# LSimon95/megatts2

Measured on AMD Instinct MI355X. Metric: mel-frames/sec (whole node), higher is better.
Workload: dtype f32; 1 GPU; C3: B=32/GPU x 1 GPU, Np=70, Tp=431, Tm=431; stages vqpe+mrte+adm+plm+decoder+vocoder; forced durations; weights=synthetic (name-seeded), parallelism=dp1 (utterance shards, one RCCL all-gather of mels per step)

## Files before the change

### megatts2_amd/csrc/capi.inc

```

namespace mt2 {
extern thread_local std::string g_last_error;
void finalize_model(mt2_model& m);
}

using namespace mt2;

#define MT2_API_BEGIN try {
#define MT2_API_END                                 \
    ::CallScope::verdict_of_open_call();            \
    return 0;                                       \
    }                                               \
    catch (const std::exception& e) {               \
        g_last_error = e.what();                    \
        return -1;                                  \
    }                                               \
    catch (...) {                                   \
        g_last_error = "unknown error";             \
        return -1;                                  \
    }

enum Need { NEED_G = 1, NEED_ADM = 2, NEED_PLM = 4, NEED_VOC = 8 };
static void require_ready(mt2_model* m, int need = 0) {
    MT2_REQUIRE(m != nullptr, "null model handle");
// ... 235 lines not shown
            f += R + 14 * R * ch;
        }
        f += R + 4ll * B + 64;
    }
    *bytes = (size_t)f * sizeof(float) + (size_t)400 * 256 + ((size_t)8 << 20);
    MT2_API_END
}

static int* option_slot(mt2_model* m, const std::string& n) {
    if (n == "ar_groups") return &m->ar_groups;
    if (n == "adm_groups") return &m->adm_groups;
    if (n == "plm_groups") return &m->plm_groups;
    if (n == "force_gemm_config") return &m->opts.force_cfg;
    if (n == "t_ks4") return &m->opts.t_ks4;
    if (n == "t_ks2") return &m->opts.t_ks2;
    if (n == "t32") return &m->opts.t32;
    if (n == "t32x32") return &m->opts.t32x32;
    if (n == "t_x6_256") return &m->opts.t_x6_256;
    if (n == "t_x6_128") return &m->opts.t_x6_128;
    if (n == "t_x3h_128") return &m->opts.t_x3h_128;
    if (n == "x3h") return &m->opts.x3h;
    if (n == "x6_ks") return &m->opts.x6_ks;
    if (n == "voc_streams") return &m->opts.voc_streams;
    if (n == "ldr_prio") return &m->opts.ldr_prio;
    if (n == "skinny_rows") return &m->opts.skinny_rows;
    if (n == "skinny_nw") return &m->opts.skinny_nw;
    if (n == "skinny_pairs") return &m->opts.skinny_pairs;
    if (n == "attn_lds_min") return &m->opts.attn_lds_min;
    if (n == "attn_x6_min") return &m->opts.attn_x6_min;
    if (n == "ln_pairs_adm") return &m->opts.ln_pairs_adm;
    if (n == "ln_pairs_maxm") return &m->opts.ln_pairs_maxm;
    if (n == "a_planes") return &m->opts.a_planes;
    return nullptr;
}
static bool* option_flag(mt2_model* m, const std::string& n) {
    if (n == "splitk") return &m->opts.splitk;
    if (n == "stage_markers") return &m->opts.markers;
    if (n == "win_conv") return &m->opts.win_conv;
    if (n == "x6_conv") return &m->opts.x6_conv;
    if (n == "x6_gemm") return &m->opts.x6_gemm;
    if (n == "skinny_tm") return &m->opts.skinny_tm;
    if (n == "ldr64") return &m->opts.ldr64;
    return nullptr;
}
int mt2_set_option(mt2_model* m, const char* name, int value) {
    MT2_API_BEGIN
// ... 935 lines not shown
```

### megatts2_amd/csrc/gemm_f32.hip

```cpp
#include "gemm_common.h"

#include <algorithm>
#include <atomic>
#include <cstdio>
#include <utility>
#include <vector>

namespace mt2 {

constexpr int LS = 36;

template <int BM, int BN, int WGM, int WGN>
__global__ __launch_bounds__(WGM* WGN * 64) void gemm_f32_kernel(GemmP p) {
    constexpr int NT = WGM * WGN * 64;
    constexpr int WTM = BM / WGM, WTN = BN / WGN;
    constexpr int TM = WTM / 32, TN = WTN / 32;
    constexpr int A_IT = BM * 8 / NT, B_IT = BN * 8 / NT;
    constexpr int ROWS_PER_IT = NT / 8;
    static_assert(BM * 8 % NT == 0 && BN * 8 % NT == 0, "tile/thread mismatch");
    static_assert(WTM % 32 == 0 && WTN % 32 == 0, "wave tile must be 32x32 MFMA tiles");

    extern __shared__ __attribute__((aligned(16))) float smem[];
    const int tid = threadIdx.x, lane = tid & 63, wave = tid >> 6;
    const int wm = wave / WGN, wn = wave % WGN;
// ... 1410 lines not shown
    { 32, 32, 512, 0, "skinny32_f32", { nullptr, nullptr, nullptr, nullptr, nullptr } },
    { 64, 32, 512, 0, "skinny64_f32", { nullptr, nullptr, nullptr, nullptr, nullptr } },
    { 32, 32, 512, 0, "skinnytm32_f32", { nullptr, nullptr, nullptr, nullptr, nullptr } },
    { 64, 32, 512, 0, "skinnytm64_f32", { nullptr, nullptr, nullptr, nullptr, nullptr } },
    MT2_RETIRED("x3hldr128x128_4x2+4_s3"),
    MT2_RETIRED("x3hldr128x128_4x2+4_s4"),
    MT2_RETIRED("x3hldr128x128_2x2+4_s3"),
    MT2_RETIRED("x3hldr128x128_2x2+4_s4"),
    MT2_X3HK(X3H_KS_32x64_K4, 32, 64, 1, 2, 4, 8, 2),
    MT2_X3HK(X3H_KS_64x64_K2, 64, 64, 2, 2, 2, 8, 3),
    MT2_X3HK(X3H_KS_32x32_K8, 32, 32, 1, 1, 8, 8, 2),
    MT2_X3HW(X3H_WIN_256x32, 1, 256, 32, 8, 1, 4, 4),
    MT2_X3HW(X3H_WIN_256x64, 2, 256, 64, 8, 1, 4, 4),
    MT2_X3HW(X3H_WIN_128x128, 4, 128, 128, 4, 2, 3, 4),
    MT2_RETIRED("x3hldr128x128_4x2+4_s4c2"),
    MT2_RETIRED("x3hldr128x128_2x2+4_s4c2"),
    MT2_X3HL(X3H_LDR_128x128, 128, 128, 4, 2, 4, 4, true),
    MT2_RETIRED("x3hldr128x128_4x2+4_s3xc"),
    MT2_RETIRED("x3hldr128x128_2x2+4_s4xc"),
};
constexpr int kSkinny32 = 87, kSkinny64 = 88, kSkinnyTm32 = 89, kSkinnyTm64 = 90;
constexpr int kNumCfgs = sizeof(kCfgs) / sizeof(kCfgs[0]);

int gemm_trace_shapes(EngineOpts& o, char* buf, int cap, int top) {
    struct Agg { int cfg, M, N, K, g; long long n; double ms, fl; };
    std::vector<Agg> v;
    for (auto& r : o.trace) {
        float dt = 0.f;
        if (hipEventSynchronize(r.e1) != hipSuccess || hipEventElapsedTime(&dt, r.e0, r.e1) != hipSuccess) return -1;
        bool found = false;
        for (auto& a : v)
            if (a.cfg == r.cfg && a.M == r.M && a.N == r.N && a.K == r.K && a.g == r.groups) {
                ++a.n; a.ms += dt; a.fl += r.flops; found = true;
                break;
            }
        if (!found) v.push_back({r.cfg, r.M, r.N, r.K, r.groups, 1, (double)dt, r.flops});
    }
    std::sort(v.begin(), v.end(), [](const Agg& a, const Agg& b) { return a.ms > b.ms; });
    int off = 0;
    for (int i = 0; i < (int)v.size() && i < top; ++i) {
        const Agg& a = v[i];
        const int w = snprintf(buf + off, cap - off, "%s %d %d %d %d %lld %.3f %.2f\n", kCfgs[a.cfg].name, a.M, a.N, a.K, a.g,
                               a.n, a.ms, a.fl / (a.ms > 0 ? a.ms : 1e-9) / 1e9);
        if (w < 0 || w >= cap - off) break;
        off += w;
    }
    return off;
}

int gemm_num_configs() { return kNumCfgs; }
const char* gemm_config_name(int idx) { return idx >= 0 && idx < kNumCfgs ? kCfgs[idx].name : ""; }

static std::atomic<unsigned long long> g_attr_done[kNumCfgs][6];

int gemm_trace_collect(EngineOpts& o, int cap, const char** names, int64_t* launches, double* flops, double* ms) {
    o.trace_on = false;
    auto& tr = o.trace;
    int n = 0;
    std::vector<std::pair<double, double>> iv;
    double fl_all = 0.0;
    bool ok = true;
    for (int i = 0; i < kNumCfgs && n < cap && ok; ++i) {
        int64_t cnt = 0;
        double fl = 0.0, t = 0.0;
        for (auto& r : tr) {
            if (r.cfg != i) continue;
            float dt = 0.f, t0 = 0.f;
            if (hipEventSynchronize(r.e1) != hipSuccess || hipEventElapsedTime(&dt, r.e0, r.e1) != hipSuccess ||
                hipEventElapsedTime(&t0, tr.front().e0, r.e0) != hipSuccess) { ok = false; break; }
            iv.emplace_back((double)t0, (double)t0 + dt);
            ++cnt; fl += r.flops; t += dt;
        }
        if (cnt == 0) continue;
        names[n] = kCfgs[i].name; launches[n] = cnt; flops[n] = fl; ms[n] = t;
        fl_all += fl;
        ++n;
    }
    if (ok && n < cap && !iv.empty()) {
        std::sort(iv.begin(), iv.end());
        double uni = 0.0, lo = iv[0].first, hi = iv[0].second;
        for (auto& x : iv) {
            if (x.first > hi) { uni += hi - lo; lo = x.first; hi = x.second; }
            else if (x.second > hi) hi = x.second;
        }
        uni += hi - lo;
        names[n] = "union"; launches[n] = (int64_t)iv.size(); flops[n] = fl_all; ms[n] = uni;
        ++n;
    }
    for (auto& r : tr) { (void)hipEventDestroy(r.e0); (void)hipEventDestroy(r.e1); }
    tr.clear();
    return ok ? n : -1;
}


static bool win_eligible(const GemmP& p) {
    return p.taps >= 2 && !p.rowbase && p.a_mul == 1 && p.groups == 1 && p.N == p.Cin &&
           (p.Cin == 32 || p.Cin == 64 || p.Cin == 128) && (p.taps - 1) * p.dil <= 64 && p.pro_act < PRO_LN;
// ... 185 lines not shown
    if (opts) { opts->last_stat_nt = p.stat_nt; opts->last_stat_w = p.stat_w; }
    const int tiles = ((p.M + c->bm - 1) / c->bm) * ((p.N + c->bn - 1) / c->bn);
    p.epi_t4 = o.epi_t4 ? 1 : 0;
    p.ldr_prio = o.ldr_prio;
    p.ldr64 = o.ldr64 ? 1 : 0;
    dim3 grid(tiles, 1, p.groups), block(c->threads);
    if (opts) opts->last_cfg = c->name;
    if (opts && opts->trace_on) {
        TraceRec r;
        r.cfg = idx;
        r.flops = 2.0 * p.M * p.N * p.K * p.groups;
        r.M = p.M; r.N = p.N; r.K = p.K; r.groups = p.groups;
        if (hipEventCreate(&r.e0) != hipSuccess || hipEventCreate(&r.e1) != hipSuccess) return hipErrorUnknown;
        (void)hipEventRecord(r.e0, s);
        hipLaunchKernelGGL(fn, grid, block, lds, s, p);
        (void)hipEventRecord(r.e1, s);
        opts->trace.push_back(r);
        return hipGetLastError();
    }
    hipLaunchKernelGGL(fn, grid, block, lds, s, p);
    return hipGetLastError();
}


}
```

### megatts2_amd/csrc/gemm_x3h.hip

```cpp
#include "gemm_common.h"

#include <atomic>

#ifndef MT2_X3H_ABLATE
#define MT2_X3H_ABLATE 0
#endif
#define MT2_ABL_NOINGEST (MT2_X3H_ABLATE == 2 || MT2_X3H_ABLATE == 5 || MT2_X3H_ABLATE == 6 || MT2_X3H_ABLATE == 7)
#define MT2_ABL_NOSPLIT (MT2_X3H_ABLATE == 3 || MT2_X3H_ABLATE == 5 || MT2_X3H_ABLATE == 6)
#define MT2_ABL_NOBARRIER (MT2_X3H_ABLATE == 6 || MT2_X3H_ABLATE == 7)
#ifdef MT2_X3H_NO_BUFFER_LOADS
#define MT2_BUFFER_LOADS false
#else
#define MT2_BUFFER_LOADS true
#endif

namespace mt2 {

typedef _Float16 f16x8 __attribute__((ext_vector_type(8)));
typedef _Float16 f16x2 __attribute__((ext_vector_type(2)));
typedef float f32x2 __attribute__((ext_vector_type(2)));
typedef unsigned u32x4 __attribute__((ext_vector_type(4)));

constexpr float kX3hLoScale = 2048.0f, kX3hLoInv = 1.0f / 2048.0f, kX3hMaxIn = 65504.0f;

// ... 735 lines not shown
    } else {
        float out[16];
#pragma unroll
        for (int e = 0; e < 16; ++e) out[e] = acc[e] * inv_s;
        if (lnx) {
            const int n = n0 + wn * 32 + (lane & 31);
            const float s_n = n < p.N ? p.ln_g[n] : 0.0f;
#pragma unroll
            for (int e = 0; e < 16; ++e) {
                const int rr = (e & 3) + 8 * (e >> 2) + 4 * half;
                out[e] = __shfl(ln_rs, rr) * (out[e] - __shfl(ln_mu, rr) * s_n);
            }
        }
        if (PRO == PRO_LNX && p.stat_out) epilogue_pre<16, PRO == PRO_LNX>(p, out, pre, g, m0 + wm * 32, n0 + wn * 32, lane, 0);
        else epilogue_pre<16>(p, out, pre, g, m0 + wm * 32, n0 + wn * 32, lane, 0);
    }
    if (probe) {
        __builtin_amdgcn_s_waitcnt(0);
        const unsigned long long t_end = __builtin_amdgcn_s_memrealtime();
        if (lane == 0) p.dbg[10] = t_end - t_loop_end;
    }
}

template <int QS, int BM, int BN, int WGM, int WGN, int NST, int PRO, int NL>
__global__ __launch_bounds__((WGM * WGN + NL) * 64) void conv_win_x3h_kernel(GemmP p) {
    constexpr int NW = WGM * WGN;
    constexpr int WTM = BM / WGM, WTN = BN / WGN;
    constexpr int TM = WTM / 32, TN = WTN / 32;
    constexpr int BPIECES = BN / 8;
    constexpr int NI = NL;
    constexpr int B_IT = (BPIECES + NI - 1) / NI;
    constexpr int STAGE_B = B_IT * NI * 1024;
    static_assert(NL > 0 && WTM % 32 == 0 && WTN % 32 == 0 && NST >= 3 && (NST - 2) * B_IT < 64 && BN == 32 * QS, "config");

    extern __shared__ __attribute__((aligned(16))) float smem[];
    const int tid = threadIdx.x, lane = tid & 63;
    const int wave_all = __builtin_amdgcn_readfirstlane(tid >> 6);
    const bool loader = wave_all >= NW;
    const int wave = loader ? wave_all - NW : wave_all;
    const int wm = wave / WGN, wn = wave % WGN;
    const int taps = p.taps, dil = p.dil;
    const int WR = BM + (taps - 1) * dil, WRp = (WR + 7) & ~7;
    char* ring = reinterpret_cast<char*>(smem);
    float* win = smem + NST * STAGE_B / 4;

    const int ntm = (p.M + BM - 1) / BM;
    const int bid = blockIdx.x;
    const int xcd = bid & 7, qq = ntm >> 3, rr = ntm & 7;
    const int tile = (xcd < rr ? xcd * (qq + 1) : rr * (qq + 1) + (xcd - rr) * qq) + (bid >> 3);
    const int m0 = tile * BM;

    const float* __restrict__ X = p.X;
    const char* __restrict__ Wh = reinterpret_cast<const char*>(p.Wh);
    const long long zoff_x = (const float*)g_zero16 - X;
    const long long zoff_w = (const char*)g_zero16 - Wh;
    const int ldx = p.ldx, Rx = p.Rx, Kt = p.K;

    {
        const int lrow = lane >> 3;
        const int ppq = WRp >> 3, pieces = QS * ppq;
        const int row_first = m0 + p.shift0;
        for (int pc = wave_all; pc < pieces; pc += NW + NL) {
            const int q = pc / ppq, r8 = pc - q * ppq;
            const int row = r8 * 8 + lrow;
            const int grow = row_first + row;
            const int slot = (lane & 7) ^ ((row >> 1) & 7);
            const bool ok = (row < WR) & ((unsigned)grow < (unsigned)Rx);
            const long long off = ok ? (long long)grow * ldx + q * 32 + slot * 4 : zoff_x;
            __builtin_amdgcn_global_load_lds((const __attribute__((address_space(1))) void*)(X + off),
                                             (__attribute__((address_space(3))) void*)(win + (q * WRp + r8 * 8) * 32), 16, 0, 0);
        }
    }
    const int nk = Kt / 32;
    long long wofs[B_IT];
#pragma unroll
    for (int j = 0; j < B_IT; ++j) {
        const int pc = j * NI + wave;
        const int n = pc * 8 + (lane >> 3);
        const int sl = (lane & 7) ^ ((n >> 1) & 7);
        wofs[j] = (pc < BPIECES && n < p.N) ? (long long)n * p.wh_ldb + sl * 16 : -1;
    }
    constexpr unsigned kOut = 0x80000000u;
    const bool fast32 = MT2_BUFFER_LOADS && !p.ldr64 && (long long)p.N * p.wh_ldb < 0x7fffffffll;
    const __amdgpu_buffer_rsrc_t rs_w = __builtin_amdgcn_make_buffer_rsrc(const_cast<char*>(Wh), 0, (int)kOut, 0x00020000);
    unsigned vob[B_IT];
#pragma unroll
    for (int j = 0; j < B_IT; ++j) vob[j] = wofs[j] >= 0 ? (unsigned)wofs[j] : kOut;
    auto issue = [&](int c, int st) __attribute__((always_inline)) {
        char* Bs = ring + st * STAGE_B + wave * 1024;
        if (fast32) {
#pragma unroll
            for (int j = 0; j < B_IT; ++j)
                __builtin_amdgcn_raw_ptr_buffer_load_lds(rs_w, (__attribute__((address_space(3))) void*)(Bs + j * NI * 1024), 16, (int)vob[j], c * 128, 0, 0);
            return;
        }
#pragma unroll
        for (int j = 0; j < B_IT; ++j) {
            const long long off = wofs[j] >= 0 ? wofs[j] + (long long)c * 128 : zoff_w;
            __builtin_amdgcn_global_load_lds((const __attribute__((address_space(1))) void*)(Wh + off),
                                             (__attribute__((address_space(3))) void*)(Bs + j * NI * 1024), 16, 0, 0);
        }
    };
    if (loader) {
        loader_priority(p.ldr_prio);
#pragma unroll
        for (int st = 0; st < NST - 1; ++st)
            if (st < nk) issue(st, st);
        if (nk >= NST - 1) wait_vmcnt<(NST - 1) * B_IT>();
        else wait_vmcnt<0>();
    } else {
        wait_vmcnt<0>();
    }
    float amax = 0.0f;
    {
        constexpr int NT = (NW + NL) * 64;
        constexpr int MAXT = (QS * (BM + 64) * 4 + NT - 1) / NT;
        const unsigned lds_w = (unsigned)(unsigned long long)(__attribute__((address_space(3))) float*)win;
        const int ntask = QS * WRp * 4;
        f32x4 in[MAXT][2];
        __builtin_amdgcn_s_barrier();
        asm volatile("" ::: "memory");
#pragma unroll
        for (int u = 0; u < MAXT; ++u) {
            const int t = tid + u * NT;
            const int tt = t < ntask ? t : 0;
            const int rbk = tt >> 2, j = tt & 3;
            const int row = rbk % WRp;
            const int swz = (row >> 1) & 7;
            const unsigned base = lds_w + (unsigned)rbk * 128;
            in[u][0] = lds_read_b128(base + (unsigned)(((2 * j) ^ swz) * 16));
            in[u][1] = lds_read_b128(base + (unsigned)(((2 * j + 1) ^ swz) * 16));
        }
        asm volatile("s_waitcnt lgkmcnt(0)" ::: "memory");
#pragma unroll
// ... 4 lines not shown
#pragma unroll
        for (int u = 0; u < MAXT; ++u) {
            const int t = tid + u * NT;
            if (t < ntask) {
                const int rbk = t >> 2, j = t & 3;
                const int row = rbk % WRp;
                const int swz = (row >> 1) & 7;
                u32x4 ph, pl;
                split2_f16<PRO>(in[u][0], in[u][1], slope0, ph, pl, amax);
                char* dst = reinterpret_cast<char*>(win) + (size_t)rbk * 128;
                *reinterpret_cast<u32x4*>(dst + ((j ^ swz) * 16)) = ph;
                *reinterpret_cast<u32x4*>(dst + (((4 + j) ^ swz) * 16)) = pl;
            }
        }
        asm volatile("s_waitcnt lgkmcnt(0)" ::: "memory");
    }
    if (p.x3h_flag != nullptr && __builtin_amdgcn_ballot_w64(amax >= kX3hMaxIn) != 0ull && lane == 0) atomicOr(p.x3h_flag, 1);
    if (loader) {
        static_assert(NST >= 3, "cross-chunk form: chunk c-1 is still being read at barrier c");
        for (int c = 0; c < nk; ++c) {
            if (c == 0) { if (NST - 2 < nk) wait_vmcnt<(NST - 2) * B_IT>(); else wait_vmcnt<0>(); }
            else if (c + NST - 3 < nk) wait_vmcnt<(NST - 3) * B_IT>();
            else wait_vmcnt<0>();
            __builtin_amdgcn_s_barrier();
            if (c >= 1 && c + NST - 2 < nk) issue(c + NST - 2, (c + NST - 2) % NST);
        }
        return;
    }
    float inv_s[TN];
#pragma unroll
    for (int j = 0; j < TN; ++j) {
        const int n = wn * WTN + j * 32 + (lane & 31);
        inv_s[j] = p.wh_inv[n < p.N ? n : 0];
    }

    f32x16 acc[TM][TN], acl[TM][TN];
#pragma unroll
    for (int i = 0; i < TM; ++i)
#pragma unroll
        for (int j = 0; j < TN; ++j)
#pragma unroll
            for (int e = 0; e < 16; ++e) { acc[i][j][e] = 0.0f; acl[i][j][e] = 0.0f; }

    const int half = lane >> 5;
    const unsigned lds_ring = (unsigned)(unsigned long long)(__attribute__((address_space(3))) char*)ring;
    const unsigned lds_win = (unsigned)(unsigned long long)(__attribute__((address_space(3))) float*)win;
    const int nrow = wn * WTN + (lane & 31);
    const unsigned b_lane = lds_ring + nrow * 128;
    const int swzb = (nrow >> 1) & 7;
    unsigned koffb[2][2];
#pragma unroll
    for (int b = 0; b < 2; ++b) {
        koffb[b][0] = (unsigned)(((b * 2 + half) ^ swzb) * 16);
        koffb[b][1] = (unsigned)(((4 + b * 2 + half) ^ swzb) * 16);
    }
    const int arow0 = wm * WTM + (lane & 31);

    constexpr int N1 = 2 * TM + 2 * TN;
    static_assert(N1 <= 15, "lgkmcnt is four bits wide");
    u32x4 ra[2][TM][2];
    u32x4 rb[2][2][TN];
    auto fetch_a = [&](int b, unsigned sa, int swza) __attribute__((always_inline)) {
        const unsigned vh = sa + (unsigned)(((b * 2 + half) ^ swza) * 16), vl = sa + (unsigned)(((4 + b * 2 + half) ^ swza) * 16);
        static_for(std::make_integer_sequence<int, TM>{}, [&](auto ic) {
            constexpr int i = decltype(ic)::value;
// ... 12 lines not shown
    auto tie_set = [&](int b) __attribute__((always_inline)) {
#pragma unroll
        for (int i = 0; i < TM; ++i) asm volatile("" : "+v"(ra[b][i][0]), "+v"(ra[b][i][1]));
#pragma unroll
        for (int pl = 0; pl < 2; ++pl)
#pragma unroll
            for (int j = 0; j < TN; ++j) asm volatile("" : "+v"(rb[b][pl][j]));
    };
    auto products = [&](int b) __attribute__((always_inline)) {
#pragma unroll
        for (int i = 0; i < TM; ++i) {
            const f16x8 Ah = __builtin_bit_cast(f16x8, ra[b][i][0]), Al = __builtin_bit_cast(f16x8, ra[b][i][1]);
#pragma unroll
            for (int j = 0; j < TN; ++j)
                acl[i][j] = __builtin_amdgcn_mfma_f32_32x32x16_f16(Ah, __builtin_bit_cast(f16x8, rb[b][1][j]), acl[i][j], 0, 0, 0);
#pragma unroll
            for (int j = 0; j < TN; ++j)
                acc[i][j] = __builtin_amdgcn_mfma_f32_32x32x16_f16(Ah, __builtin_bit_cast(f16x8, rb[b][0][j]), acc[i][j], 0, 0, 0);
#pragma unroll
            for (int j = 0; j < TN; ++j)
                acl[i][j] = __builtin_amdgcn_mfma_f32_32x32x16_f16(Al, __builtin_bit_cast(f16x8, rb[b][0][j]), acl[i][j], 0, 0, 0);
        }
    };
    __builtin_amdgcn_s_barrier();
    asm volatile("" ::: "memory");
    {
        const unsigned sa0 = lds_win + (unsigned)(arow0 * BK) * 4;
        const int swz0 = (arow0 >> 1) & 7;
        fetch_a(0, sa0, swz0); fetch_b(0, b_lane); fetch_a(1, sa0, swz0); fetch_b(1, b_lane);
    }
    __builtin_amdgcn_sched_barrier(0);
    int stn = 1 % NST, tapn = 0, qn = 1;
    if (qn == QS) { qn = 0; tapn = 1; }
    auto chunk = [&](auto last_c) __attribute__((always_inline)) {
        constexpr bool last = decltype(last_c)::value;
        const int arow = arow0 + tapn * dil;
        const int swza = (arow >> 1) & 7;
        const unsigned sa = lds_win + (unsigned)((qn * WRp + arow) * BK) * 4;
        const unsigned sb = b_lane + (unsigned)stn * STAGE_B;
#pragma unroll
        for (int b = 0; b < 2; ++b) {
            if (last && b == 1) asm volatile("s_waitcnt lgkmcnt(0)" ::: "memory");
            else asm volatile("s_waitcnt lgkmcnt(%0)" :: "n"(N1) : "memory");
            tie_set(b);
            __builtin_amdgcn_sched_barrier(0);
            products(b);
            __builtin_amdgcn_sched_barrier(0);
            if constexpr (!last) {
                if (b == 0) {
                    __builtin_amdgcn_s_barrier();
                    asm volatile("" ::: "memory");
                }
                fetch_a(b, sa, swza);
                fetch_b(b, sb);
                __builtin_amdgcn_sched_barrier(0);
            }
        }
        stn = stn + 1 == NST ? 0 : stn + 1;
        if (++qn == QS) { qn = 0; ++tapn; }
    };
    for (int c = 0; c + 1 < nk; ++c) chunk(std::false_type{});
    chunk(std::true_type{});
#pragma unroll
    for (int i = 0; i < TM; ++i)
#pragma unroll
        for (int j = 0; j < TN; ++j)
#pragma unroll
            for (int e = 0; e < 16; ++e) acc[i][j][e] = __builtin_fmaf(acl[i][j][e], kX3hLoInv, acc[i][j][e]) * inv_s[j];
    if (epilogue_t4_ok(p)) epilogue_t4<TM, TN>(p, acc, 0, m0 + wm * WTM, wn * WTN, lane);
    else epilogue<TM, TN>(p, acc, 0, m0 + wm * WTM, wn * WTN, lane);
}

#define MT2_X3H_LDR(BM_, BN_, WM_, WN_, NL_, NST_)                                                                          \
    { gemm_x3h_ldr_kernel<BM_, BN_, WM_, WN_, NL_, NST_, ACT_NONE>, gemm_x3h_ldr_kernel<BM_, BN_, WM_, WN_, NL_, NST_, ACT_RELU>, \
      gemm_x3h_ldr_kernel<BM_, BN_, WM_, WN_, NL_, NST_, ACT_LRELU>, gemm_x3h_ldr_kernel<BM_, BN_, WM_, WN_, NL_, NST_, PRO_APL>, nullptr, \
      gemm_x3h_ldr_kernel<BM_, BN_, WM_, WN_, NL_, NST_, PRO_LNX> }
#define MT2_X3H_KS(BM_, BN_, WM_, WN_, KS_, NL_, NST_)                                                                          \
    { gemm_x3h_ks_kernel<BM_, BN_, WM_, WN_, KS_, NL_, NST_, ACT_NONE>, gemm_x3h_ks_kernel<BM_, BN_, WM_, WN_, KS_, NL_, NST_, ACT_RELU>, \
      gemm_x3h_ks_kernel<BM_, BN_, WM_, WN_, KS_, NL_, NST_, ACT_LRELU>, gemm_x3h_ks_kernel<BM_, BN_, WM_, WN_, KS_, NL_, NST_, PRO_APL>, nullptr, \
      gemm_x3h_ks_kernel<BM_, BN_, WM_, WN_, KS_, NL_, NST_, PRO_LNX> }

#define MT2_X3H_WIN(QS_, BM_, BN_, WM_, WN_, NST_, NL_)                                                                         \
    { conv_win_x3h_kernel<QS_, BM_, BN_, WM_, WN_, NST_, ACT_NONE, NL_>, conv_win_x3h_kernel<QS_, BM_, BN_, WM_, WN_, NST_, ACT_RELU, NL_>, \
      conv_win_x3h_kernel<QS_, BM_, BN_, WM_, WN_, NST_, ACT_LRELU, NL_>, nullptr, nullptr, nullptr }

X3hKernel x3h_kernel(int tile, int variant) {
    static void (*const kTable[kX3hTiles][6])(GemmP) = {
        MT2_X3H_LDR(128, 128, 4, 2, 4, 4),
        MT2_X3H_KS(32, 64, 1, 2, 4, 8, 2),
        MT2_X3H_KS(64, 64, 2, 2, 2, 8, 3),
        MT2_X3H_KS(32, 32, 1, 1, 8, 8, 2),
        MT2_X3H_WIN(2, 256, 64, 8, 1, 4, 4),
        MT2_X3H_WIN(4, 128, 128, 4, 2, 3, 4),
        MT2_X3H_WIN(1, 256, 32, 8, 1, 4, 4),
    };
    if (tile < 0 || tile >= kX3hTiles || variant < 0 || variant >= 6) return nullptr;
    return kTable[tile][variant];
}

}
```

### megatts2_amd/csrc/model_stages.hip

```cpp
#include "mt2_model.h"
#include "x3h_planes.h"

#include <algorithm>
#include <cmath>
#include <cstring>
#include <numeric>

namespace mt2 {



static RowSet make_rows(const int* lens, int B, int G) {
    RowSet rs;
    rs.B = B; rs.G = G;
    rs.len.assign(lens, lens + B);
    rs.off.resize(B);
    int r = G;
    for (int b = 0; b < B; ++b) {
        MT2_REQUIRE(lens[b] >= 0, "negative utterance length");
        rs.off[b] = r;
        r += lens[b] + G;
        rs.maxlen = std::max(rs.maxlen, lens[b]);
    }
    rs.R = r;
// ... 151 lines not shown
    }
    const bool planes = linear_takes_planes(c, h_scratch, K, M, w.W, w.bias, N, K, y, ldy, epi_act);
    LnP q{};
    q.x = x + (long long)shift0 * ldx; q.ldx = ldx * p.a_mul; q.gamma = w.g; q.beta = w.b; q.out = h_scratch; q.ldo = K;
    q.M = M; q.C = K; q.eps = 1e-5f; q.act = ACT_NONE; q.out_planes = planes ? 1 : 0; q.x3h_flag = c.m.opts.x3h_flag;
    MT2_HIP(launch_layernorm(q, c.s));
    linear(c, h_scratch, K, M, w.W, w.bias, N, K, y, ldy, nullptr, 0, nullptr, epi_act, planes, c_planes);
}
static LnOps ln1_qkv(const EncLayerW& w, int d, int n0 = 0) {
    return ln_ops(w.ln1g, w.ln1b, w.wqkv, w.bqkv, w.wqkv_l, w.sqkv, w.cqkv, n0, d);
}
static LnOps ln2_ff0(const EncLayerW& w, int d) {
    return ln_ops(w.ln2g, w.ln2b, w.ff0w, w.ff0b, w.ff0_l, w.sff0, w.cff0, 0, d);
}

static void conv_same(const Ctx& c, const float* x, int ldx, int R, const ConvW& w, float* y, int ldy,
                      const int* valid, int pro_act = ACT_NONE, float slope = 0.f, int epi_act = ACT_NONE,
                      const float* Rsd = nullptr, int ldr = 0, int dil = 1) {
    GemmP p{};
    p.X = x; p.ldx = ldx; p.Rx = R; p.taps = w.k; p.dil = dil; p.shift0 = -((w.k - 1) / 2) * dil; p.Cin = w.cin;
    p.W = w.w; p.bias = w.b; p.R = Rsd; p.ldr = ldr; p.valid = valid; p.C = y; p.ldc = ldy; p.M = R; p.N = w.cout;
    p.pro_act = pro_act; p.pro_slope = slope; p.epi_act = epi_act;
    gemm(c, p);
}

static void layernorm(const Ctx& c, const float* x, int ldx, const float* g, const float* b, int M, int C,
                      float* out, int ldo, const int* valid = nullptr, int valid_rows = 0,
                      const float* R1 = nullptr, int ldr1 = 0, int r1_rows = 0, int rows_per_group = 0,
                      int act = ACT_NONE, bool out_planes = false) {
    LnP p{};
    p.x = x; p.ldx = ldx; p.gamma = g; p.beta = b; p.rows_per_group = rows_per_group;
    p.R1 = R1; p.ldr1 = ldr1; p.r1_rows = r1_rows; p.valid = valid; p.valid_rows = valid_rows;
    p.out = out; p.ldo = ldo; p.M = M; p.C = C; p.eps = 1e-5f; p.act = act;
    p.out_planes = out_planes ? 1 : 0; p.x3h_flag = c.m.opts.x3h_flag;
    MT2_HIP(launch_layernorm(p, c.s));
}

static float* run_stack(const Ctx& c, const StackW& w, const float* x_in, bool shared_in, int R,
                        const int* valid) {
    const int C = w.C, G = w.groups;
    const size_t per = (size_t)R * C;
    float* T = c.ws.get<float>(per * G);
    float* Y = c.ws.get<float>(per * G);
    float* XA = c.ws.get<float>(per * G);
    float* XB = c.ws.get<float>(per * G);
    const float* cur = x_in;
// ... 983 lines not shown
        MT2_REQUIRE(cfg.hg_n_res == 3, "HiFi-GAN V1 uses three resblocks per stage");
        const int nside = m.opts.voc_streams > 1 ? 2 : 0;
        ensure_aux(m, nside);
        if (reflect) {
            int g0 = 0;
            for (int j = 0; j < 3; ++j) g0 = std::max(g0, (m.hg_res[i * 3 + j].k - 1) / 2 * m.hg_res[i * 3 + j].dil[0]);
            halo(c, up, ch, g0);
        }
        if (nside) {
            MT2_HIP(hipEventRecord(m.ev_fork, c.s));
            m.aux_forked = true;
            for (int j = 0; j < nside; ++j) MT2_HIP(hipStreamWaitEvent(m.aux_streams[j], m.ev_fork, 0));
        }
        for (int j = 0; j < 3; ++j) {
            const ResW& r = m.hg_res[i * 3 + j];
            const Ctx cj{m, (nside && j > 0) ? m.aux_streams[j - 1] : c.s, c.ws};
            float* t1 = c.ws.get<float>(per);
            float* ha = c.ws.get<float>(per);
            float* hb = c.ws.get<float>(per);
            rb[j] = c.ws.get<float>(per);
            const float* h = up;
            for (int n = 0; n < 3; ++n) {
                float* out = n == 2 ? rb[j] : (n == 0 ? ha : hb);
                if (n > 0) halo(cj, const_cast<float*>(h), ch, (r.k - 1) / 2 * r.dil[n]);
                conv_same(cj, h, ch, (int)R, r.c1[n], t1, ch, valid, ACT_LRELU, slope, ACT_LRELU, nullptr, 0, r.dil[n]);
                halo(cj, t1, ch, (r.k - 1) / 2);
                conv_same(cj, t1, ch, (int)R, r.c2[n], out, ch, valid, ACT_NONE, slope, ACT_NONE, h, ch, 1);
                h = out;
            }
        }
        for (int j = 0; j < nside; ++j) {
            MT2_HIP(hipEventRecord(m.ev_join[j], m.aux_streams[j]));
            MT2_HIP(hipStreamWaitEvent(c.s, m.ev_join[j], 0));
        }
        if (!reflect && i + 1 == cfg.hg_n_up && m.hg_post.cout == 1 && (ch & 3) == 0 && ch <= 128 && m.hg_post.k <= 15) {
            float* wav = c.ws.get<float>((size_t)R);
            const hipError_t e = launch_conv_post(rb[0], rb[1], rb[2], 1.0f / 3.0f, R, ch, m.hg_post.k, m.hg_post.w,
                                                  m.hg_post.b, 0.01f, valid, wav, c.s);
            if (e == hipSuccess) return wav;
            if (e != hipErrorNotSupported) MT2_HIP(e);
        }
        x = c.ws.get<float>(per);
        MT2_HIP(launch_avg3(rb[0], rb[1], rb[2], 1.0f / 3.0f, x, (long long)per, c.s));
    }
    float* wav = c.ws.get<float>((size_t)R);
    halo(c, x, ch, (m.hg_post.k - 1) / 2);
// ... 103 lines not shown
```

### megatts2_amd/csrc/mt2_kernels.h

```cpp
#pragma once
#include <hip/hip_runtime.h>
#include <stdint.h>

#include <atomic>
#include <vector>

namespace mt2 {

inline hipError_t dyn_lds_once(std::atomic<unsigned long long>& done, const void* fn, size_t bytes) {
    int dev = 0;
    hipError_t e = hipGetDevice(&dev);
    if (e != hipSuccess) return e;
    const unsigned long long bit = 1ull << (dev & 63);
    if (done.load(std::memory_order_acquire) & bit) return hipSuccess;
    e = hipFuncSetAttribute(fn, hipFuncAttributeMaxDynamicSharedMemorySize, (int)bytes);
    if (e != hipSuccess) return e;
    done.fetch_or(bit, std::memory_order_release);
    return hipSuccess;
}

constexpr int kInvalidRow = -(1 << 30);

enum Act : int { ACT_NONE = 0, ACT_RELU = 1, ACT_LRELU = 2, ACT_TANH = 3,
                 ACT_LOGCLAMP = 4 };
// ... 17 lines not shown
    const float* wh_inv = nullptr;
    long long wh_inv_stride = 0;
    int* x3h_flag = nullptr;
    const float* Wtm = nullptr;
    int tm_n0 = 0, tm_k0 = 0;
    int tm_kb = 0;
    const float* bias; long long strideB;
    const float* R; long long strideR; int ldr;
    const int* valid;
    float* C; long long strideC; int ldc;
    int M, N, K, groups;
    int pro_act; float pro_slope; int epi_act; float out_scale;
    const float* ln_g; const float* ln_b; float ln_eps;
    float* stat_out = nullptr; int stat_nt = 0, stat_w = 0;
    const float* ln_stat = nullptr; int ln_nt = 0, ln_w = 0;
};
struct TraceRec { int cfg; double flops; hipEvent_t e0, e1; int M, N, K, groups; };
struct EngineOpts {
    int force_cfg = -1;
    int t_ks4 = 256, t_ks2 = 640, t32 = 64, t32x32 = 160;
    bool splitk = true;
    int voc_streams = 3;
    bool win_conv = true;
    bool x6_conv = true;
    bool x6_gemm = true;
    bool x6_splitk = true;
    int x3h = 15;
    int* x3h_flag = nullptr;
    int t_x3h_128 = 72;
    int t_x6_256 = 160, t_x6_128 = 72;
    int x6_ks = 4;
    bool epi_t4 = true;
    int a_planes = 3;
    bool ldr64 = false;
    int ldr_prio = 3;
    int skinny_rows = 64;
    int attn_lds_min = 640;
    int attn_x6_min = 192;
    int attn_lds_waves = 0;
    int attn_ds = 1;
    bool skinny_tm = true;
    int skinny_groups = 1;
    int skinny_pairs = 1;
    int skinny_nw = 16;
    bool markers = false;
    bool trace_on = false;
    std::vector<TraceRec> trace;
    const char* last_cfg = "";
    int last_stat_nt = 0, last_stat_w = 0;
    int ln_pairs = 0;
    int ln_pairs_adm = 2;
    int ln_pairs_maxk = 1024;
    int ln_pairs_maxm = 1280;
};
hipError_t launch_gemm(const GemmP& p, hipStream_t s, EngineOpts* o = nullptr);
bool gemm_takes_planes(const GemmP& p, const EngineOpts& o);
bool gemm_writes_planes(const GemmP& p, const EngineOpts& o);
enum X3hTile : int { X3H_LDR_128x128 = 0, X3H_KS_32x64_K4, X3H_KS_64x64_K2, X3H_KS_32x32_K8, X3H_WIN_256x64, X3H_WIN_128x128, X3H_WIN_256x32, kX3hTiles };
typedef void (*X3hKernel)(GemmP);
X3hKernel x3h_kernel(int tile, int variant);
bool gemm_skinny_eligible(const GemmP& p, int max_rows);
hipError_t launch_gemm_skinny(const GemmP& p, hipStream_t s);
bool gemm_skinny_tm_eligible(const GemmP& p, int max_rows);
hipError_t launch_gemm_skinny_tm(const GemmP& p, hipStream_t s);
hipError_t launch_tile_major(const float* W, int N, int K, float* out, hipStream_t s);
int gemm_num_configs();
const char* gemm_config_name(int idx);
int gemm_trace_collect(EngineOpts& o, int cap, const char** names, int64_t* launches, double* flops, double* ms);
int gemm_trace_shapes(EngineOpts& o, char* buf, int cap, int top);

struct LnP {
    const float* x; int ldx;
    const float* gamma; const float* beta; int rows_per_group;
    const float* R1; int ldr1; int r1_rows; const float* R2; int ldr2;
    const int* valid; int valid_rows;
    float* out; int ldo;
    int M, C; float eps; int act;
    int out_planes = 0;
    int* x3h_flag = nullptr;
};
hipError_t launch_layernorm(const LnP& p, hipStream_t s);

struct LnReduceP {
// ... 88 lines not shown
```

Measured before the change: 78590 mel-frames/s.

## Fuse vocoder resblock conv pairs into one windowed x3h kernel

```diff
diff --git a/megatts2_amd/csrc/capi.inc b/megatts2_amd/csrc/capi.inc
--- a/megatts2_amd/csrc/capi.inc
+++ b/megatts2_amd/csrc/capi.inc
@@ -281,6 +281,7 @@
     if (n == "x3h") return &m->opts.x3h;
     if (n == "x6_ks") return &m->opts.x6_ks;
     if (n == "voc_streams") return &m->opts.voc_streams;
+    if (n == "voc_fuse") return &m->opts.voc_fuse;
     if (n == "ldr_prio") return &m->opts.ldr_prio;
     if (n == "skinny_rows") return &m->opts.skinny_rows;
     if (n == "skinny_nw") return &m->opts.skinny_nw;
diff --git a/megatts2_amd/csrc/gemm_f32.hip b/megatts2_amd/csrc/gemm_f32.hip
--- a/megatts2_amd/csrc/gemm_f32.hip
+++ b/megatts2_amd/csrc/gemm_f32.hip
@@ -1456,6 +1456,10 @@
 constexpr int kSkinny32 = 87, kSkinny64 = 88, kSkinnyTm32 = 89, kSkinnyTm64 = 90;
 constexpr int kNumCfgs = sizeof(kCfgs) / sizeof(kCfgs[0]);
 
+static const char* const kPairNames[] = {"x3hrbp256x32_8x1+4_s4", "x3hrbp256x64_8x1+4_s4", "x3hrbp128x128_4x2+4_s3"};
+constexpr int kNumPair = sizeof(kPairNames) / sizeof(kPairNames[0]), kNumTraced = kNumCfgs + kNumPair;
+static const char* traced_name(int cfg) { return cfg < kNumCfgs ? kCfgs[cfg].name : kPairNames[cfg - kNumCfgs]; }
+
 int gemm_trace_shapes(EngineOpts& o, char* buf, int cap, int top) {
     struct Agg { int cfg, M, N, K, g; long long n; double ms, fl; };
     std::vector<Agg> v;
@@ -1474,7 +1478,7 @@
     int off = 0;
     for (int i = 0; i < (int)v.size() && i < top; ++i) {
         const Agg& a = v[i];
-        const int w = snprintf(buf + off, cap - off, "%s %d %d %d %d %lld %.3f %.2f\n", kCfgs[a.cfg].name, a.M, a.N, a.K, a.g,
+        const int w = snprintf(buf + off, cap - off, "%s %d %d %d %d %lld %.3f %.2f\n", traced_name(a.cfg), a.M, a.N, a.K, a.g,
                                a.n, a.ms, a.fl / (a.ms > 0 ? a.ms : 1e-9) / 1e9);
         if (w < 0 || w >= cap - off) break;
         off += w;
@@ -1494,7 +1498,7 @@
     std::vector<std::pair<double, double>> iv;
     double fl_all = 0.0;
     bool ok = true;
-    for (int i = 0; i < kNumCfgs && n < cap && ok; ++i) {
+    for (int i = 0; i < kNumTraced && n < cap && ok; ++i) {
         int64_t cnt = 0;
         double fl = 0.0, t = 0.0;
         for (auto& r : tr) {
@@ -1506,7 +1510,7 @@
             ++cnt; fl += r.flops; t += dt;
         }
         if (cnt == 0) continue;
-        names[n] = kCfgs[i].name; launches[n] = cnt; flops[n] = fl; ms[n] = t;
+        names[n] = traced_name(i); launches[n] = cnt; flops[n] = fl; ms[n] = t;
         fl_all += fl;
         ++n;
     }
@@ -1738,5 +1742,56 @@
     return hipGetLastError();
 }
 
-
+static std::atomic<unsigned long long> g_pair_attr_done[kNumPair];
+hipError_t launch_resblock_pair(const GemmP& c1, const GemmP& c2, hipStream_t s, EngineOpts* opts) {
+    static const EngineOpts kDefaults;
+    const EngineOpts& o = opts ? *opts : kDefaults;
+    if (c1.M <= 0) return hipSuccess;
+    if (!o.voc_fuse || !(o.x3h & 4) || !o.win_conv || !o.x6_conv || o.force_cfg >= 0) return hipErrorNotSupported;
+    GemmP p1 = c1, p2 = c2;
+    for (GemmP* p : {&p1, &p2}) {
+        if (p->wh_ldb == 0) p->wh_ldb = 4ll * ((p->ldw + 31) / 32 * 32);
+        if (!win_eligible(*p) || !p->W3 || !p->Wh || !p->wh_inv || p->K != p->taps * p->Cin || (p->K & 31) || (p->ldw & 7) ||
+            (((unsigned long long)p->Wh) & 127) || (p->wh_ldb & 127) || p->a_planes || p->c_planes || p->stat_out)
+            return hipErrorNotSupported;
+    }
+    const int k = p1.taps, ch = p1.Cin;
+    const bool shapes = p2.taps == k && p2.Cin == ch && (k & 1) && p2.dil == 1 && p1.M == p2.M && p1.Rx == p1.M &&
+                        p1.shift0 == -((k - 1) / 2) * p1.dil && p1.ldx == ch && p2.R == p1.X && p2.ldr == p1.ldx && p1.valid == p2.valid &&
+                        p1.pro_act == ACT_LRELU && p1.epi_act == ACT_LRELU && p1.R == nullptr && p2.epi_act == ACT_NONE &&
+                        p2.out_scale == 1.0f && p2.wh_ldb == p1.wh_ldb && p2.C != p1.X && (long long)p1.N * p1.wh_ldb < 0x7fffffffll;
+    if (!shapes) return hipErrorNotSupported;
+    const int idx = ch == 32 ? 98 : (ch == 64 ? 99 : 100), pi = idx - 98;
+    const TileCfg* c = &kCfgs[idx];
+    void (*fn)(GemmP, GemmP) = x3h_pair_kernel(c->win_qs);
+    if (!fn || c->win_qs * 32 != ch || k - 1 >= c->bm) return hipErrorNotSupported;
+    const size_t wrp = (size_t)((c->bm + (k - 1) * p1.dil + 7) & ~7), wrp_max = (size_t)((c->bm + 64 + 7) & ~7);
+    const size_t lds = c->lds + (size_t)c->win_qs * wrp * BK * sizeof(float) + (size_t)c->bm * sizeof(int);
+    const size_t lds_attr = c->lds + (size_t)c->win_qs * wrp_max * BK * sizeof(float) + (size_t)c->bm * sizeof(int);
+    hipError_t e = dyn_lds_once(g_pair_attr_done[pi], reinterpret_cast<const void*>(fn), lds_attr);
+    if (e != hipSuccess) return e;
+    p1.x3h_flag = p2.x3h_flag = o.x3h_flag;
+    p1.epi_t4 = p2.epi_t4 = o.epi_t4 ? 1 : 0;
+    p1.ldr_prio = p2.ldr_prio = o.ldr_prio;
+    p1.ldr64 = p2.ldr64 = o.ldr64 ? 1 : 0;
+    const int bm2 = c->bm - (k - 1);
+    const int tiles = (p1.M + bm2 - 1) / bm2;
+    dim3 grid(tiles), block(c->threads);
+    if (opts) opts->last_cfg = kPairNames[pi];
+    if (opts && opts->trace_on) {
+        TraceRec r;
+        r.cfg = kNumCfgs + pi;
+        r.flops = 2.0 * 2.0 * (double)tiles * c->bm * p1.N * p1.K;
+        r.M = p1.M; r.N = p1.N; r.K = p1.K; r.groups = 1;
+        if (hipEventCreate(&r.e0) != hipSuccess || hipEventCreate(&r.e1) != hipSuccess) return hipErrorUnknown;
+        (void)hipEventRecord(r.e0, s);
+        hipLaunchKernelGGL(fn, grid, block, lds, s, p1, p2);
+        (void)hipEventRecord(r.e1, s);
+        opts->trace.push_back(r);
+        return hipGetLastError();
+    }
+    hipLaunchKernelGGL(fn, grid, block, lds, s, p1, p2);
+    return hipGetLastError();
 }
+
+}
diff --git a/megatts2_amd/csrc/gemm_x3h.hip b/megatts2_amd/csrc/gemm_x3h.hip
--- a/megatts2_amd/csrc/gemm_x3h.hip
+++ b/megatts2_amd/csrc/gemm_x3h.hip
@@ -781,8 +781,8 @@
     }
 }
 
-template <int QS, int BM, int BN, int WGM, int WGN, int NST, int PRO, int NL>
-__global__ __launch_bounds__((WGM * WGN + NL) * 64) void conv_win_x3h_kernel(GemmP p) {
+template <int QS, int BM, int BN, int WGM, int WGN, int NST, int PRO, int NL, bool PAIR>
+__device__ __forceinline__ void conv_win_x3h_body(const GemmP& p, const GemmP& p2) {
     constexpr int NW = WGM * WGN;
     constexpr int WTM = BM / WGM, WTN = BN / WGN;
     constexpr int TM = WTM / 32, TN = WTN / 32;
@@ -803,17 +803,27 @@
     char* ring = reinterpret_cast<char*>(smem);
     float* win = smem + NST * STAGE_B / 4;
 
-    const int ntm = (p.M + BM - 1) / BM;
+    const int BM2 = PAIR ? BM - (taps - 1) : BM;
+    const int ntm = (p.M + BM2 - 1) / BM2;
     const int bid = blockIdx.x;
     const int xcd = bid & 7, qq = ntm >> 3, rr = ntm & 7;
     const int tile = (xcd < rr ? xcd * (qq + 1) : rr * (qq + 1) + (xcd - rr) * qq) + (bid >> 3);
-    const int m0 = tile * BM;
+    const int o0 = tile * BM2;
+    const int m0 = PAIR ? o0 - (taps - 1) / 2 : o0;
 
     const float* __restrict__ X = p.X;
     const char* __restrict__ Wh = reinterpret_cast<const char*>(p.Wh);
+    const char* __restrict__ Wh2 = reinterpret_cast<const char*>(PAIR ? p2.Wh : p.Wh);
     const long long zoff_x = (const float*)g_zero16 - X;
-    const long long zoff_w = (const char*)g_zero16 - Wh;
     const int ldx = p.ldx, Rx = p.Rx, Kt = p.K;
+    [[maybe_unused]] int* vrow = reinterpret_cast<int*>(smem + NST * STAGE_B / 4 + QS * WRp * 32);
+    [[maybe_unused]] int vr = 0;
+    if constexpr (PAIR) {
+        if (tid < BM) {
+            const int gr = m0 + tid;
+            vr = (unsigned)gr < (unsigned)p.M ? (p.valid ? p.valid[gr] : 1) : 0;
+        }
+    }
 
     {
         const int lrow = lane >> 3;
@@ -830,7 +840,7 @@
                                              (__attribute__((address_space(3))) void*)(win + (q * WRp + r8 * 8) * 32), 16, 0, 0);
         }
     }
-    const int nk = Kt / 32;
+    const int nk1 = Kt / 32, nk = PAIR ? 2 * nk1 : nk1;
     long long wofs[B_IT];
 #pragma unroll
     for (int j = 0; j < B_IT; ++j) {
@@ -842,21 +852,27 @@
     constexpr unsigned kOut = 0x80000000u;
     const bool fast32 = MT2_BUFFER_LOADS && !p.ldr64 && (long long)p.N * p.wh_ldb < 0x7fffffffll;
     const __amdgpu_buffer_rsrc_t rs_w = __builtin_amdgcn_make_buffer_rsrc(const_cast<char*>(Wh), 0, (int)kOut, 0x00020000);
+    [[maybe_unused]] const __amdgpu_buffer_rsrc_t rs_w2 = __builtin_amdgcn_make_buffer_rsrc(const_cast<char*>(Wh2), 0, (int)kOut, 0x00020000);
     unsigned vob[B_IT];
 #pragma unroll
     for (int j = 0; j < B_IT; ++j) vob[j] = wofs[j] >= 0 ? (unsigned)wofs[j] : kOut;
     auto issue = [&](int c, int st) __attribute__((always_inline)) {
         char* Bs = ring + st * STAGE_B + wave * 1024;
+        const bool second = PAIR && c >= nk1;
+        const int cw = second ? c - nk1 : c;
         if (fast32) {
 #pragma unroll
             for (int j = 0; j < B_IT; ++j)
-                __builtin_amdgcn_raw_ptr_buffer_load_lds(rs_w, (__attribute__((address_space(3))) void*)(Bs + j * NI * 1024), 16, (int)vob[j], c * 128, 0, 0);
+                __builtin_amdgcn_raw_ptr_buffer_load_lds(second ? rs_w2 : rs_w, (__attribute__((address_space(3))) void*)(Bs + j * NI * 1024), 16,
+                                                         (int)vob[j], cw * 128, 0, 0);
             return;
         }
+        const char* __restrict__ Wc = second ? Wh2 : Wh;
+        const long long zoff_w = (const char*)g_zero16 - Wc;
 #pragma unroll
         for (int j = 0; j < B_IT; ++j) {
-            const long long off = wofs[j] >= 0 ? wofs[j] + (long long)c * 128 : zoff_w;
-            __builtin_amdgcn_global_load_lds((const __attribute__((address_space(1))) void*)(Wh + off),
+            const long long off = wofs[j] >= 0 ? wofs[j] + (long long)cw * 128 : zoff_w;
+            __builtin_amdgcn_global_load_lds((const __attribute__((address_space(1))) void*)(Wc + off),
                                              (__attribute__((address_space(3))) void*)(Bs + j * NI * 1024), 16, 0, 0);
         }
     };
@@ -869,6 +885,10 @@
         else wait_vmcnt<0>();
     } else {
         wait_vmcnt<0>();
+        if constexpr (PAIR) {
+            static_assert(BM <= NW * 64, "one row mask per compute thread");
+            if (tid < BM) vrow[tid] = vr;
+        }
     }
     float amax = 0.0f;
     {
@@ -919,25 +939,21 @@
             if (c == 0) { if (NST - 2 < nk) wait_vmcnt<(NST - 2) * B_IT>(); else wait_vmcnt<0>(); }
             else if (c + NST - 3 < nk) wait_vmcnt<(NST - 3) * B_IT>();
             else wait_vmcnt<0>();
+            if (PAIR && c == nk1) __builtin_amdgcn_s_barrier();
             __builtin_amdgcn_s_barrier();
             if (c >= 1 && c + NST - 2 < nk) issue(c + NST - 2, (c + NST - 2) % NST);
         }
         return;
     }
-    float inv_s[TN];
+    float inv_s[TN], inv_s2[PAIR ? TN : 1];
 #pragma unroll
     for (int j = 0; j < TN; ++j) {
         const int n = wn * WTN + j * 32 + (lane & 31);
         inv_s[j] = p.wh_inv[n < p.N ? n : 0];
+        if constexpr (PAIR) inv_s2[j] = p2.wh_inv[n < p.N ? n : 0];
     }
 
     f32x16 acc[TM][TN], acl[TM][TN];
-#pragma unroll
-    for (int i = 0; i < TM; ++i)
-#pragma unroll
-        for (int j = 0; j < TN; ++j)
-#pragma unroll
-            for (int e = 0; e < 16; ++e) { acc[i][j][e] = 0.0f; acl[i][j][e] = 0.0f; }
 
     const int half = lane >> 5;
     const unsigned lds_ring = (unsigned)(unsigned long long)(__attribute__((address_space(3))) char*)ring;
@@ -996,54 +1012,122 @@
                 acl[i][j] = __builtin_amdgcn_mfma_f32_32x32x16_f16(Al, __builtin_bit_cast(f16x8, rb[b][0][j]), acl[i][j], 0, 0, 0);
         }
     };
-    __builtin_amdgcn_s_barrier();
-    asm volatile("" ::: "memory");
-    {
-        const unsigned sa0 = lds_win + (unsigned)(arow0 * BK) * 4;
-        const int swz0 = (arow0 >> 1) & 7;
-        fetch_a(0, sa0, swz0); fetch_b(0, b_lane); fetch_a(1, sa0, swz0); fetch_b(1, b_lane);
-    }
-    __builtin_amdgcn_sched_barrier(0);
-    int stn = 1 % NST, tapn = 0, qn = 1;
-    if (qn == QS) { qn = 0; tapn = 1; }
-    auto chunk = [&](auto last_c) __attribute__((always_inline)) {
-        constexpr bool last = decltype(last_c)::value;
-        const int arow = arow0 + tapn * dil;
-        const int swza = (arow >> 1) & 7;
-        const unsigned sa = lds_win + (unsigned)((qn * WRp + arow) * BK) * 4;
-        const unsigned sb = b_lane + (unsigned)stn * STAGE_B;
-#pragma unroll
-        for (int b = 0; b < 2; ++b) {
-            if (last && b == 1) asm volatile("s_waitcnt lgkmcnt(0)" ::: "memory");
-            else asm volatile("s_waitcnt lgkmcnt(%0)" :: "n"(N1) : "memory");
-            tie_set(b);
-            __builtin_amdgcn_sched_barrier(0);
-            products(b);
-            __builtin_amdgcn_sched_barrier(0);
-            if constexpr (!last) {
-                if (b == 0) {
-                    __builtin_amdgcn_s_barrier();
-                    asm volatile("" ::: "memory");
+    auto conv_k = [&](int wrp, int dl, int c0, int nkc, const float (&inv)[TN]) __attribute__((always_inline)) {
+#pragma unroll
+        for (int i = 0; i < TM; ++i)
+#pragma unroll
+            for (int j = 0; j < TN; ++j)
+#pragma unroll
+                for (int e = 0; e < 16; ++e) { acc[i][j][e] = 0.0f; acl[i][j][e] = 0.0f; }
+        __builtin_amdgcn_s_barrier();
+        asm volatile("" ::: "memory");
+        const int st0 = c0 % NST;
+        {
+            const unsigned sa0 = lds_win + (unsigned)(arow0 * BK) * 4;
+            const int swz0 = (arow0 >> 1) & 7;
+            const unsigned sb0 = b_lane + (unsigned)st0 * STAGE_B;
+            fetch_a(0, sa0, swz0); fetch_b(0, sb0); fetch_a(1, sa0, swz0); fetch_b(1, sb0);
+        }
+        __builtin_amdgcn_sched_barrier(0);
+        int stn = st0 + 1 == NST ? 0 : st0 + 1, tapn = 0, qn = 1;
+        if (qn == QS) { qn = 0; tapn = 1; }
+        auto chunk = [&](auto last_c) __attribute__((always_inline)) {
+            constexpr bool last = decltype(last_c)::value;
+            const int arow = arow0 + tapn * dl;
+            const int swza = (arow >> 1) & 7;
+            const unsigned sa = lds_win + (unsigned)((qn * wrp + arow) * BK) * 4;
+            const unsigned sb = b_lane + (unsigned)stn * STAGE_B;
+#pragma unroll
+            for (int b = 0; b < 2; ++b) {
+                if (last && b == 1) asm volatile("s_waitcnt lgkmcnt(0)" ::: "memory");
+                else asm volatile("s_waitcnt lgkmcnt(%0)" :: "n"(N1) : "memory");
+                tie_set(b);
+                __builtin_amdgcn_sched_barrier(0);
+                products(b);
+                __builtin_amdgcn_sched_barrier(0);
+                if constexpr (!last) {
+                    if (b == 0) {
+                        __builtin_amdgcn_s_barrier();
+                        asm volatile("" ::: "memory");
+                    }
+                    fetch_a(b, sa, swza);
+                    fetch_b(b, sb);
+                    __builtin_amdgcn_sched_barrier(0);
                 }
-                fetch_a(b, sa, swza);
-                fetch_b(b, sb);
-                __builtin_amdgcn_sched_barrier(0);
-            }
-        }
-        stn = stn + 1 == NST ? 0 : stn + 1;
-        if (++qn == QS) { qn = 0; ++tapn; }
+            }
+            stn = stn + 1 == NST ? 0 : stn + 1;
+            if (++qn == QS) { qn = 0; ++tapn; }
+        };
+        for (int c = 0; c + 1 < nkc; ++c) chunk(std::false_type{});
+        chunk(std::true_type{});
+#pragma unroll
+        for (int i = 0; i < TM; ++i)
+#pragma unroll
+            for (int j = 0; j < TN; ++j)
+#pragma unroll
+                for (int e = 0; e < 16; ++e) acc[i][j][e] = __builtin_fmaf(acl[i][j][e], kX3hLoInv, acc[i][j][e]) * inv[j];
     };
-    for (int c = 0; c + 1 < nk; ++c) chunk(std::false_type{});
-    chunk(std::true_type{});
-#pragma unroll
-    for (int i = 0; i < TM; ++i)
-#pragma unroll
-        for (int j = 0; j < TN; ++j)
-#pragma unroll
-            for (int e = 0; e < 16; ++e) acc[i][j][e] = __builtin_fmaf(acl[i][j][e], kX3hLoInv, acc[i][j][e]) * inv_s[j];
-    if (epilogue_t4_ok(p)) epilogue_t4<TM, TN>(p, acc, 0, m0 + wm * WTM, wn * WTN, lane);
-    else epilogue<TM, TN>(p, acc, 0, m0 + wm * WTM, wn * WTN, lane);
+    conv_k(WRp, dil, 0, nk1, inv_s);
+    if constexpr (PAIR) {
+        const int WR2p = (BM + taps - 1 + 7) & ~7;
+        float bv[TN];
+#pragma unroll
+        for (int j = 0; j < TN; ++j) {
+            const int n = wn * WTN + j * 32 + (lane & 31);
+            bv[j] = p.bias ? p.bias[n < p.N ? n : 0] : 0.0f;
+        }
+        __builtin_amdgcn_s_barrier();
+        asm volatile("" ::: "memory");
+        int vm[TM][16];
+#pragma unroll
+        for (int i = 0; i < TM; ++i)
+#pragma unroll
+            for (int e = 0; e < 16; ++e) vm[i][e] = vrow[wm * WTM + i * 32 + (e & 3) + 8 * (e >> 2) + 4 * half];
+        const int epi_act = p.epi_act, cl = lane & 31;
+        const float epi_par = p.pro_slope, out_scale = p.out_scale;
+        float amax2 = 0.0f;
+        char* t1 = reinterpret_cast<char*>(win);
+#pragma unroll
+        for (int j = 0; j < TN; ++j) {
+            const int qb = (wn * WTN + j * 32) >> 5;
+#pragma unroll
+            for (int i = 0; i < TM; ++i)
+#pragma unroll
+                for (int e = 0; e < 16; ++e) {
+                    const int r = wm * WTM + i * 32 + (e & 3) + 8 * (e >> 2) + 4 * half;
+                    float v = act_rt(epi_act, acc[i][j][e] + bv[j], epi_par) * out_scale;
+                    if (vm[i][e] == 0) v = 0.0f;
+                    amax2 = fmaxf(fabsf(v), amax2);
+                    const _Float16 h = (_Float16)v;
+                    const _Float16 l = (_Float16)__builtin_fmaf((float)h, -kX3hLoScale, v * kX3hLoScale);
+                    const int swz = (r >> 1) & 7;
+                    char* blk = t1 + (size_t)(qb * WR2p + r) * 128 + (cl & 7) * 2;
+                    *reinterpret_cast<_Float16*>(blk + (((cl >> 3) ^ swz) * 16)) = h;
+                    *reinterpret_cast<_Float16*>(blk + ((((cl >> 3) + 4) ^ swz) * 16)) = l;
+                }
+        }
+        asm volatile("s_waitcnt lgkmcnt(0)" ::: "memory");
+        if (p.x3h_flag != nullptr && __builtin_amdgcn_ballot_w64(amax2 >= kX3hMaxIn) != 0ull && lane == 0) atomicOr(p.x3h_flag, 1);
+        conv_k(WR2p, 1, nk1, nk1, inv_s2);
+        GemmP q = p2;
+        q.M = min(p2.M, o0 + BM2);
+        if (epilogue_t4_ok(q)) epilogue_t4<TM, TN>(q, acc, 0, o0 + wm * WTM, wn * WTN, lane);
+        else epilogue<TM, TN>(q, acc, 0, o0 + wm * WTM, wn * WTN, lane);
+    } else {
+        if (epilogue_t4_ok(p)) epilogue_t4<TM, TN>(p, acc, 0, m0 + wm * WTM, wn * WTN, lane);
+        else epilogue<TM, TN>(p, acc, 0, m0 + wm * WTM, wn * WTN, lane);
+    }
 }
+
+template <int QS, int BM, int BN, int WGM, int WGN, int NST, int PRO, int NL>
+__global__ __launch_bounds__((WGM * WGN + NL) * 64) void conv_win_x3h_kernel(GemmP p) {
+    conv_win_x3h_body<QS, BM, BN, WGM, WGN, NST, PRO, NL, false>(p, p);
+}
+template <int QS, int BM, int BN, int WGM, int WGN, int NST, int NL>
+__global__ __launch_bounds__((WGM * WGN + NL) * 64) void conv_pair_x3h_kernel(GemmP p1, GemmP p2) {
+    conv_win_x3h_body<QS, BM, BN, WGM, WGN, NST, ACT_LRELU, NL, true>(p1, p2);
+}
+
 
 #define MT2_X3H_LDR(BM_, BN_, WM_, WN_, NL_, NST_)                                                                          \
     { gemm_x3h_ldr_kernel<BM_, BN_, WM_, WN_, NL_, NST_, ACT_NONE>, gemm_x3h_ldr_kernel<BM_, BN_, WM_, WN_, NL_, NST_, ACT_RELU>, \
@@ -1072,4 +1156,13 @@
     return kTable[tile][variant];
 }
 
+X3hPairKernel x3h_pair_kernel(int qs) {
+    switch (qs) {
+        case 1: return conv_pair_x3h_kernel<1, 256, 32, 8, 1, 4, 4>;
+        case 2: return conv_pair_x3h_kernel<2, 256, 64, 8, 1, 4, 4>;
+        case 4: return conv_pair_x3h_kernel<4, 128, 128, 4, 2, 3, 4>;
+        default: return nullptr;
+    }
 }
+
+}
diff --git a/megatts2_amd/csrc/model_stages.hip b/megatts2_amd/csrc/model_stages.hip
--- a/megatts2_amd/csrc/model_stages.hip
+++ b/megatts2_amd/csrc/model_stages.hip
@@ -197,6 +197,22 @@
     p.W = w.w; p.bias = w.b; p.R = Rsd; p.ldr = ldr; p.valid = valid; p.C = y; p.ldc = ldy; p.M = R; p.N = w.cout;
     p.pro_act = pro_act; p.pro_slope = slope; p.epi_act = epi_act;
     gemm(c, p);
+}
+
+static bool resblock_pair(const Ctx& c, const float* h, int ch, int R, const ConvW& w1, const ConvW& w2, int dil, float slope,
+                          float* out, const int* valid) {
+    if (!c.m.opts.voc_fuse) return false;
+    GemmP p1{}, p2{};
+    p1.X = h; p1.ldx = ch; p1.Rx = R; p1.taps = w1.k; p1.dil = dil; p1.shift0 = -((w1.k - 1) / 2) * dil; p1.Cin = w1.cin;
+    p1.W = w1.w; p1.bias = w1.b; p1.valid = valid; p1.M = R; p1.N = w1.cout;
+    p1.pro_act = ACT_LRELU; p1.pro_slope = slope; p1.epi_act = ACT_LRELU;
+    p2.X = nullptr; p2.ldx = ch; p2.Rx = R; p2.taps = w2.k; p2.dil = 1; p2.shift0 = -((w2.k - 1) / 2); p2.Cin = w2.cin;
+    p2.W = w2.w; p2.bias = w2.b; p2.R = h; p2.ldr = ch; p2.valid = valid; p2.C = out; p2.ldc = ch; p2.M = R; p2.N = w2.cout;
+    p2.pro_act = ACT_NONE; p2.pro_slope = slope; p2.epi_act = ACT_NONE;
+    const hipError_t e = launch_resblock_pair(planned(c, p1), planned(c, p2), c.s, &c.m.opts);
+    if (e == hipSuccess) return true;
+    if (e != hipErrorNotSupported) MT2_HIP(e);
+    return false;
 }
 
 static void layernorm(const Ctx& c, const float* x, int ldx, const float* g, const float* b, int M, int C,
@@ -1226,6 +1242,10 @@
             const float* h = up;
             for (int n = 0; n < 3; ++n) {
                 float* out = n == 2 ? rb[j] : (n == 0 ? ha : hb);
+                if (!reflect && resblock_pair(cj, h, ch, (int)R, r.c1[n], r.c2[n], r.dil[n], slope, out, valid)) {
+                    h = out;
+                    continue;
+                }
                 if (n > 0) halo(cj, const_cast<float*>(h), ch, (r.k - 1) / 2 * r.dil[n]);
                 conv_same(cj, h, ch, (int)R, r.c1[n], t1, ch, valid, ACT_LRELU, slope, ACT_LRELU, nullptr, 0, r.dil[n]);
                 halo(cj, t1, ch, (r.k - 1) / 2);
diff --git a/megatts2_amd/csrc/mt2_kernels.h b/megatts2_amd/csrc/mt2_kernels.h
--- a/megatts2_amd/csrc/mt2_kernels.h
+++ b/megatts2_amd/csrc/mt2_kernels.h
@@ -63,6 +63,7 @@
     bool splitk = true;
     int voc_streams = 3;
     bool win_conv = true;
+    int voc_fuse = 1;
     bool x6_conv = true;
     bool x6_gemm = true;
     bool x6_splitk = true;
@@ -100,6 +101,9 @@
 enum X3hTile : int { X3H_LDR_128x128 = 0, X3H_KS_32x64_K4, X3H_KS_64x64_K2, X3H_KS_32x32_K8, X3H_WIN_256x64, X3H_WIN_128x128, X3H_WIN_256x32, kX3hTiles };
 typedef void (*X3hKernel)(GemmP);
 X3hKernel x3h_kernel(int tile, int variant);
+typedef void (*X3hPairKernel)(GemmP, GemmP);
+X3hPairKernel x3h_pair_kernel(int qs);
+hipError_t launch_resblock_pair(const GemmP& c1, const GemmP& c2, hipStream_t s, EngineOpts* o);
 bool gemm_skinny_eligible(const GemmP& p, int max_rows);
 hipError_t launch_gemm_skinny(const GemmP& p, hipStream_t s);
 bool gemm_skinny_tm_eligible(const GemmP& p, int max_rows);
```

New measurement: 79670 mel-frames/s (median of 6 runs). +1.4%, better.
